# matvogel/P2P-Bridge

Hardware: AMD Instinct MI355X
Metric: denoised points/sec (8192-pt patches, T=30) (higher is better)
Workload: dtype f32; 1 GPU; PVDS_PUNet xyz-only, 8192-pt patches, T=30 bridge steps, batch 32 per GPU (BASELINE configs[1]); patches_per_gpu=32, points_per_patch=8192, bridge_steps=30, parallelism=patch-shard x1, process_group_world_size=1, hipgraph=True, weights=seeded random init (26.44 M params)

## Files before the change

### p2p_bridge_amd/csrc/common.h

```cpp
#pragma once
#include <hip/hip_runtime.h>
#include <stdint.h>
#include <type_traits>

#include "../../include/p2pb_hip.h"

#define P2PB_WAVE 64

static inline int p2pb_launch_status() { return (int)hipGetLastError(); }
int p2pb_split_terms_now();
#define p2pb_g_split_terms (p2pb_split_terms_now())

static inline unsigned cdiv(long a, long b) { return (unsigned)((a + b - 1) / b); }

template <int... Vs, class F>
static inline int for_value(int v, F &&f) {
  int rc = P2PB_EINVAL;
  (void)((v == Vs && (rc = f(std::integral_constant<int, Vs>{}), true)) || ...);
  return rc;
}
template <class F>
static inline int for_flag(bool v, F &&f) {
  return v ? f(std::true_type{}) : f(std::false_type{});
}

__device__ __forceinline__ float sqdist3(float dx, float dy, float dz) {
  return __fmaf_rn(dz, dz, __fmaf_rn(dy, dy, dx * dx));
}

__device__ __forceinline__ int lane_id() { return (int)(threadIdx.x & 63); }

__device__ __forceinline__ int mbcnt(unsigned long long mask) {
  return (int)__builtin_amdgcn_mbcnt_hi((unsigned)(mask >> 32), __builtin_amdgcn_mbcnt_lo((unsigned)mask, 0u));
}

template <int CTRL, int ROW_MASK>
__device__ __forceinline__ float dpp_add_step(float v) {
  const int o = __builtin_amdgcn_update_dpp(0, __builtin_bit_cast(int, v), CTRL, ROW_MASK, 0xf, false);
  return v + __builtin_bit_cast(float, o);
}
__device__ __forceinline__ float halfwave_sum_to_last(float v) {
  v = dpp_add_step<0x111, 0xf>(v);
  v = dpp_add_step<0x112, 0xf>(v);
  v = dpp_add_step<0x114, 0xf>(v);
  v = dpp_add_step<0x118, 0xf>(v);
  v = dpp_add_step<0x142, 0xa>(v);
  return v;
}

typedef __bf16 bf16x8 __attribute__((ext_vector_type(8)));
typedef __bf16 bf16x2 __attribute__((ext_vector_type(2)));
typedef float f32x2 __attribute__((ext_vector_type(2)));
typedef unsigned u32x4 __attribute__((ext_vector_type(4)));
typedef float f32x16 __attribute__((ext_vector_type(16)));

__device__ __forceinline__ void split3(float a, float b, unsigned &p0, unsigned &p1, unsigned &p2) {
  f32x2 v = {a, b};
  const bf16x2 q0 = __builtin_convertvector(v, bf16x2);
  v = v - __builtin_convertvector(q0, f32x2);
  const bf16x2 q1 = __builtin_convertvector(v, bf16x2);
  v = v - __builtin_convertvector(q1, f32x2);
  const bf16x2 q2 = __builtin_convertvector(v, bf16x2);
  p0 = __builtin_bit_cast(unsigned, q0);
  p1 = __builtin_bit_cast(unsigned, q1);
  p2 = __builtin_bit_cast(unsigned, q2);
}

#define SPLIT_BF16X6 6
#define SPLIT_BF16X3 3
#define SPLIT_F16X3 16
#define SPLIT_F16_SX 4.0f
typedef _Float16 f16x8 __attribute__((ext_vector_type(8)));
typedef _Float16 f16x2 __attribute__((ext_vector_type(2)));
__device__ __forceinline__ void split2h(float a, float b, unsigned &p0, unsigned &p1) {
  f32x2 v = {a, b};
  const f16x2 q0 = __builtin_convertvector(v, f16x2);
  v = v - __builtin_convertvector(q0, f32x2);
  const f16x2 q1 = __builtin_convertvector(v, f16x2);
  p0 = __builtin_bit_cast(unsigned, q0);
  p1 = __builtin_bit_cast(unsigned, q1);
}
template <int MODE>
__device__ __forceinline__ void split_pair(float a, float b, unsigned &p0, unsigned &p1, unsigned &p2) {
  if constexpr (MODE == SPLIT_F16X3) {
    split2h(a * SPLIT_F16_SX, b * SPLIT_F16_SX, p0, p1);
    p2 = 0u;
  } else {
    split3(a, b, p0, p1, p2);
  }
}
#define SPLIT_X2W_FLAG 0x100
#ifdef P2PB_X2W_TIMING
#define X2W_KEEP_LOW_WEIGHT_PRODUCT 0
#else
#define X2W_KEEP_LOW_WEIGHT_PRODUCT 1
#endif
constexpr __host__ __device__ int split_planes(int mode) { return mode == SPLIT_BF16X6 ? 3 : 2; }
template <int MODE>
__device__ __forceinline__ f32x16 split_mfma(const u32x4 &a, const u32x4 &b, const f32x16 &c) {
  if constexpr (MODE == SPLIT_F16X3)
    return __builtin_amdgcn_mfma_f32_32x32x16_f16(__builtin_bit_cast(f16x8, a), __builtin_bit_cast(f16x8, b), c, 0, 0, 0);
  else
    return __builtin_amdgcn_mfma_f32_32x32x16_bf16(__builtin_bit_cast(bf16x8, a), __builtin_bit_cast(bf16x8, b), c, 0, 0, 0);
}
__device__ __forceinline__ float f16_weight_scale(float wmax) {
  if (!(wmax > 0.0f) || wmax > 3.0e38f) return 1.0f;
  int e;
  (void)frexpf(wmax, &e);
  return ldexpf(1.0f, 14 - e);
}
struct GnFinish {
  const float *gamma, *beta, *style;
  float *scale, *shift, *chmean;
  double count_per_channel;
  int style_stride, groups;
  float eps;
};
static inline bool gn_shape_ok(int c, int groups, const float *style, int style_stride) {
  return groups > 0 && c % groups == 0 && c / groups <= 256 && !(style && style_stride < 2 * c);
}
typedef float gnf_f32x2 __attribute__((ext_vector_type(2)));
__device__ __forceinline__ void gn_finish_group_v(int c, int nslots, const float *__restrict__ part, const GnFinish &f, int b, int g,
                                                  double *lds, int vt, bool live, float *mean_rstd = nullptr,
                                                  float *tab_scale = nullptr, float *tab_shift = nullptr, float *tab_mean = nullptr) {
  double *rs = lds, *rq = lds + 256, *chs = lds + 512, *chq = lds + 768;
  const int t = vt;
  const int cg = c / f.groups, g0 = g * cg;
  const int nt = 256 / cg;
  const int k = t % cg, j = t / cg;
  float p_ga = 1.0f, p_be = 0.0f, p_fa = 1.0f, p_bi = 0.0f;
  if (live && t < cg) {
    const int ch = g0 + t;
    if (f.gamma) p_ga = f.gamma[ch];
    if (f.beta) p_be = f.beta[ch];
    if (f.style) {
      p_fa = f.style[(size_t)b * f.style_stride + ch];
      p_bi = f.style[(size_t)b * f.style_stride + c + ch];
    }
  }
  double s = 0.0, q = 0.0;
  if (live && j < nt) {
    const float *p0 = part + ((size_t)b * nslots * c + g0 + k) * 2;
    const size_t pitch = (size_t)c * 2;
    int sl = j;
    for (; sl + 7 * nt < nslots; sl += 8 * nt) {
      gnf_f32x2 v[8];
#pragma unroll
      for (int u = 0; u < 8; ++u) {
        const float *pp = p0 + (size_t)(sl + u * nt) * pitch;
        v[u] = *(const gnf_f32x2 *)pp;
      }
#pragma unroll
      for (int u = 0; u < 8; ++u) {
        s += (double)v[u][0];
        q += (double)v[u][1];
      }
    }
    for (; sl + 3 * nt < nslots; sl += 4 * nt) {
      gnf_f32x2 v[4];
#pragma unroll
      for (int u = 0; u < 4; ++u) {
        const float *pp = p0 + (size_t)(sl + u * nt) * pitch;
        v[u] = *(const gnf_f32x2 *)pp;
      }
#pragma unroll
      for (int u = 0; u < 4; ++u) {
        s += (double)v[u][0];
        q += (double)v[u][1];
      }
    }
    for (; sl < nslots; sl += nt) {
      const float *p = p0 + (size_t)sl * pitch;
      s += (double)p[0];
      q += (double)p[1];
    }
  }
  if (live) {
    rs[t] = s;
    rq[t] = q;
  }
  __syncthreads();
  if (live && t < cg) {
    double ts = 0.0, tq = 0.0;
    for (int jj = 0; jj < nt; ++jj) {
      ts += rs[jj * cg + t];
      tq += rq[jj * cg + t];
    }
    chs[t] = ts;
    chq[t] = tq;
  }
  __syncthreads();
  if (live && t < cg) {
    double gs = 0.0, gq = 0.0;
    for (int kk = 0; kk < cg; ++kk) {
      gs += chs[kk];
      gq += chq[kk];
    }
    const int ch = g0 + t;
    const double n = f.count_per_channel * cg;
    const double mean = gs / n;
    double var = gq / n - mean * mean;
    if (var < 0.0) var = 0.0;
    const double rstd = 1.0 / sqrt(var + (double)f.eps);
    const double ga = (double)p_ga, be = (double)p_be, fa = (double)p_fa, bi = (double)p_bi;
    const double sc = rstd * ga * fa;
    const double sh = (be - mean * rstd * ga) * fa + bi;
    const float cm = (float)(sc * (chs[t] / f.count_per_channel) + sh);
    if (f.scale) f.scale[(size_t)b * c + ch] = (float)sc;
    if (f.shift) f.shift[(size_t)b * c + ch] = (float)sh;
    if (f.chmean) f.chmean[(size_t)b * c + ch] = cm;
    if (tab_scale) tab_scale[ch] = (float)sc;
    if (tab_shift) tab_shift[ch] = (float)sh;
    if (tab_mean) tab_mean[ch] = cm;
    if (mean_rstd && t == 0) {
      mean_rstd[((size_t)b * f.groups + g) * 2] = (float)mean;
      mean_rstd[((size_t)b * f.groups + g) * 2 + 1] = (float)rstd;
    }
  }
  __syncthreads();
}
__device__ __forceinline__ void gn_finish_group(int c, int nslots, const float *__restrict__ part, const GnFinish &f, int b, int g,
                                                double *lds, float *mean_rstd = nullptr) {
  gn_finish_group_v(c, nslots, part, f, b, g, lds, (int)threadIdx.x, threadIdx.x < 256, mean_rstd);
}
template <int NS>
__device__ __forceinline__ void gn_finish_sample(int c, int nslots, const float *__restrict__ part, const GnFinish &f, int b, double *lds,
                                                 float *tab_scale = nullptr, float *tab_shift = nullptr, float *tab_mean = nullptr) {
  const int slice = (int)threadIdx.x >> 8, vt = (int)threadIdx.x & 255;
  for (int g0 = 0; g0 < f.groups; g0 += NS) {
    const int g = g0 + slice;
    gn_finish_group_v(c, nslots, part, f, b, g < f.groups ? g : 0, lds + slice * 1024, vt, slice < NS && g < f.groups, nullptr,
                      tab_scale, tab_shift, tab_mean);
  }
}
template <int CTRL>
__device__ __forceinline__ float dpp_full(float v) {
  const int i = __builtin_bit_cast(int, v);
  return __builtin_bit_cast(float, __builtin_amdgcn_update_dpp(i, i, CTRL, 0xf, 0xf, false));
}
__device__ __forceinline__ void permlane16_swap(float &a, float &b) {
  asm volatile("s_nop 1\n\tv_permlane16_swap_b32 %0, %1\n\ts_nop 1" : "+v"(a), "+v"(b));
}
struct RowAdd {
  __device__ static float f(float a, float b) { return a + b; }
};
__device__ __forceinline__ float vmin_raw(float a, float b) {
  float r;
  asm("v_min_f32 %0, %1, %2" : "=v"(r) : "v"(a), "v"(b));
  return r;
}
__device__ __forceinline__ float vmax_raw(float a, float b) {
  float r;
  asm("v_max_f32 %0, %1, %2" : "=v"(r) : "v"(a), "v"(b));
  return r;
}
struct RowMin {
  __device__ static float f(float a, float b) {
    float r;
    asm("v_min_f32 %0, %1, %2" : "=v"(r) : "v"(a), "v"(b));
    return r;
  }
};
struct RowMax {
  __device__ static float f(float a, float b) {
    float r;
    asm("v_max_f32 %0, %1, %2" : "=v"(r) : "v"(a), "v"(b));
    return r;
  }
};
template <class Op>
__device__ __forceinline__ float rowreduce32(float (&v)[32]) {
  const int lane = (int)(threadIdx.x & 63);
#pragma unroll
  for (int i = 0; i < 16; ++i) {
    float a = v[i], b = v[i + 16];
    permlane16_swap(a, b);
    v[i] = Op::f(a, b);
  }
#pragma unroll
  for (int i = 0; i < 8; ++i) {
    const float x = Op::f(v[i], dpp_full<0x128>(v[i])), y = Op::f(v[i + 8], dpp_full<0x128>(v[i + 8]));
    v[i] = (lane & 8) ? y : x;
  }
#pragma unroll
  for (int i = 0; i < 4; ++i) {
    const float x = Op::f(v[i], dpp_full<0x141>(v[i])), y = Op::f(v[i + 4], dpp_full<0x141>(v[i + 4]));
    v[i] = (lane & 4) ? y : x;
  }
#pragma unroll
  for (int i = 0; i < 2; ++i) {
    const float x = Op::f(v[i], dpp_full<0x4E>(v[i])), y = Op::f(v[i + 2], dpp_full<0x4E>(v[i + 2]));
    v[i] = (lane & 2) ? y : x;
  }
  const float x = Op::f(v[0], dpp_full<0xB1>(v[0])), y = Op::f(v[1], dpp_full<0xB1>(v[1]));
  return (lane & 1) ? y : x;
}

template <class Op>
__device__ __forceinline__ void groupreduce8(float (&v)[32]) {
  const int lane = (int)(threadIdx.x & 63);
#pragma unroll
  for (int i = 0; i < 16; ++i) {
    const float x = Op::f(v[i], dpp_full<0x141>(v[i])), y = Op::f(v[i + 16], dpp_full<0x141>(v[i + 16]));
    v[i] = (lane & 4) ? y : x;
  }
#pragma unroll
  for (int i = 0; i < 8; ++i) {
    const float x = Op::f(v[i], dpp_full<0x4E>(v[i])), y = Op::f(v[i + 8], dpp_full<0x4E>(v[i + 8]));
    v[i] = (lane & 2) ? y : x;
  }
#pragma unroll
  for (int i = 0; i < 4; ++i) {
    const float x = Op::f(v[i], dpp_full<0xB1>(v[i])), y = Op::f(v[i + 4], dpp_full<0xB1>(v[i + 4]));
    v[i] = (lane & 1) ? y : x;
  }
}

template <class Op>
__device__ __forceinline__ void groupreduce16(float (&v)[32]) {
  const int lane = (int)(threadIdx.x & 63);
#pragma unroll
  for (int i = 0; i < 16; ++i) {
    const float x = Op::f(v[i], dpp_full<0x140>(v[i])), y = Op::f(v[i + 16], dpp_full<0x140>(v[i + 16]));
    v[i] = (lane & 8) ? y : x;
  }
#pragma unroll
  for (int i = 0; i < 8; ++i) {
    const float x = Op::f(v[i], dpp_full<0x141>(v[i])), y = Op::f(v[i + 8], dpp_full<0x141>(v[i + 8]));
    v[i] = (lane & 4) ? y : x;
  }
#pragma unroll
  for (int i = 0; i < 4; ++i) {
    const float x = Op::f(v[i], dpp_full<0x4E>(v[i])), y = Op::f(v[i + 4], dpp_full<0x4E>(v[i + 4]));
    v[i] = (lane & 2) ? y : x;
  }
#pragma unroll
  for (int i = 0; i < 2; ++i) {
    const float x = Op::f(v[i], dpp_full<0xB1>(v[i])), y = Op::f(v[i + 2], dpp_full<0xB1>(v[i + 2]));
    v[i] = (lane & 1) ? y : x;
  }
}

enum {
  P2PB_FORM_PW_FP32 = 0,
  P2PB_FORM_PW_WIDE_FP32 = 1,
  P2PB_FORM_PW_WIDE_F16 = 2,
  P2PB_FORM_PW_SPLIT128 = 3,
  P2PB_FORM_PW_SPLIT256 = 4,
  P2PB_FORM_PW_PINGPONG = 5,
  P2PB_FORM_PW_GATHER = 6,
};
void p2pb_note_pointwise_form(int cin, int cout, int npos, int form);
int p2pb_gn_affine_launch(int b, int c, int nslots, const float *part, const GnFinish &f, hipStream_t s);

long p2pb_experiment_long(const char *key, long dflt);

int p2pb_zero_async(void *p, size_t nbytes, hipStream_t s);

bool p2pb_deterministic();
```

### p2p_bridge_amd/csrc/pointwise.hip

```cpp
#include "pw_common.h"
#include "absmax.h"

__global__ void pw_pack_kernel(int cout, int cin, int cin_pad, int cout_pad, const float *__restrict__ w,
                               float *__restrict__ wp, long s_co, long s_ci) {
  const size_t total = (size_t)cin_pad * cout_pad;
  for (size_t e = (size_t)blockIdx.x * 256 + threadIdx.x; e < total; e += (size_t)gridDim.x * 256) {
    const int kk = (int)(e & 3);
    const int co = (int)((e >> 2) % cout_pad);
    const int kh = (int)((e / ((size_t)4 * cout_pad)) & 1);
    const int chunk = (int)(e / ((size_t)8 * cout_pad));
    const int ci = chunk * 8 + 2 * kk + kh;
    wp[e] = (co < cout && ci < cin) ? w[(size_t)co * s_co + (size_t)ci * s_ci] : 0.0f;
  }
}

extern "C" size_t p2pb_pointwise_packed_floats(int cout, int cin) {
  return (size_t)pw_cin_pad(cin) * pw_cout_pad(cout);
}

static int pw_pack(int cout, int cin, const float *w, float *wp, bool adjoint, void *stream) {
  if (cout <= 0 || cin <= 0) return P2PB_EINVAL;
  const size_t total = p2pb_pointwise_packed_floats(cout, cin);
  hipLaunchKernelGGL(pw_pack_kernel, dim3((unsigned)((total + 255) / 256 > 2048 ? 2048 : (total + 255) / 256)), dim3(256),
                     0, (hipStream_t)stream, cout, cin, pw_cin_pad(cin), pw_cout_pad(cout), w, wp, adjoint ? 1L : (long)cin,
                     adjoint ? (long)cout : 1L);
  return p2pb_launch_status();
}
extern "C" int p2pb_pointwise_pack_weights(int cout, int cin, const float *w, float *wp, void *stream) {
  return pw_pack(cout, cin, w, wp, false, stream);
}
extern "C" int p2pb_pointwise_pack_weights_adjoint(int cout, int cin, const float *w_forward, float *wp, void *stream) {
  return pw_pack(cout, cin, w_forward, wp, true, stream);
}

__global__ void pw_pack_split_kernel(int cout, int cin, int nchunk, int ncoblk, const float *__restrict__ w,
                                     unsigned short *__restrict__ wp, int mode, float *__restrict__ trailer, long s_co, long s_ci,
                                     const unsigned *__restrict__ amax) {
  const size_t total = (size_t)nchunk * ncoblk * 2 * 2 * 128 * 8;
  const bool x2w = (mode & SPLIT_X2W_FLAG) != 0;
  mode &= 0xff;
  const float wmax = amax ? __builtin_bit_cast(float, *amax) : trailer[0];
  const float sw = mode == SPLIT_F16X3 ? f16_weight_scale(wmax) : 1.0f;
  if (blockIdx.x == 0 && threadIdx.x == 0) {
    trailer[1] = mode == SPLIT_F16X3 ? 1.0f / (SPLIT_F16_SX * sw) : 1.0f;
    if (amax) trailer[0] = wmax, trailer[2] = trailer[3] = 0.0f;
  }
  for (size_t e = (size_t)blockIdx.x * 256 + threadIdx.x; e < total; e += (size_t)gridDim.x * 256) {
    const int idx = (int)(e & 7);
    size_t q = e >> 3;
    const int col = (int)(q & 127);
    q >>= 7;
    const int kh = (int)(q & 1);
    q >>= 1;
    const int ks = (int)(q & 1);
    q >>= 1;
    const int cb = (int)(q % ncoblk), chunk = (int)(q / ncoblk);
    const int co = cb * 128 + col, ci = chunk * PWS_CK + ks * 16 + kh * 8 + idx;
    const float x = (co < cout && ci < cin) ? w[(size_t)co * s_co + (size_t)ci * s_ci] : 0.0f;
    unsigned p0, p1, p2;
    if (mode == SPLIT_F16X3) {
      split2h(x * sw, 0.0f, p0, p1);
      if (x2w) p1 = 0u;
      p2 = 0u;
    } else {
      split3(x, 0.0f, p0, p1, p2);
    }
    const unsigned pp[3] = {p0, p1, p2};
    for (int s = 0; s < 3; ++s)
      wp[((((((size_t)chunk * ncoblk + cb) * 2 + ks) * 3 + s) * 2 + kh) * 128 + col) * 8 + idx] = (unsigned short)(pp[s] & 0xffff);
  }
}

extern "C" size_t p2pb_pointwise_split_packed_bytes(int cout, int cin) {
  const size_t nchunk = (cin + PWS_CK - 1) / PWS_CK, ncoblk = (cout + 127) / 128;
  return nchunk * ncoblk * (2 * 3 * 2 * 128) * 16 + 16;
}

static int pw_pack_split(int cout, int cin, const float *w, void *wp, bool adjoint, void *stream, const unsigned *amax = nullptr) {
  if (cout <= 0 || cin <= 0) return P2PB_EINVAL;
  const int nchunk = (cin + PWS_CK - 1) / PWS_CK, ncoblk = (cout + 127) / 128;
  const size_t total = (size_t)nchunk * ncoblk * 2 * 2 * 128 * 8;
  float *trailer = (float *)((char *)wp + (size_t)nchunk * ncoblk * PWS_TILE * 16);
  static const long x2w = p2pb_experiment_long("x2w", 0);
  const int mode = p2pb_g_split_terms;
  if (mode == SPLIT_F16X3 && !amax) {
    const int rc = p2pb_zero_async(trailer, 16, (hipStream_t)stream);
    if (rc) return rc;
    hipLaunchKernelGGL(absmax_bits_kernel, dim3(absmax_blocks((size_t)cout * cin)), dim3(256), 0, (hipStream_t)stream, w, (size_t)cout * cin,
                       (unsigned *)trailer);
  }
  hipLaunchKernelGGL(pw_pack_split_kernel, dim3((unsigned)((total + 255) / 256 > 2048 ? 2048 : (total + 255) / 256)),
                     dim3(256), 0, (hipStream_t)stream, cout, cin, nchunk, ncoblk, w, (unsigned short *)wp,
                     mode | ((x2w && mode == SPLIT_F16X3 && !adjoint) ? SPLIT_X2W_FLAG : 0), trailer,
                     adjoint ? 1L : (long)cin, adjoint ? (long)cout : 1L, mode == SPLIT_F16X3 ? amax : nullptr);
  return p2pb_launch_status();
}
extern "C" int p2pb_pointwise_pack_weights_split(int cout, int cin, const float *w, void *wp, void *stream) {
  return pw_pack_split(cout, cin, w, wp, false, stream);
}
extern "C" int p2pb_pointwise_pack_weights_split_adjoint(int cout, int cin, const float *w_forward, void *wp, void *stream) {
  return pw_pack_split(cout, cin, w_forward, wp, true, stream);
}
extern "C" int p2pb_pointwise_pack_weights_split_amax(int cout, int cin, const float *w, void *wp, const unsigned *amax_bits,
                                                      void *stream) {
  return amax_bits ? pw_pack_split(cout, cin, w, wp, false, stream, amax_bits) : P2PB_EINVAL;
}

static GnFinish pw_fin(double count_per_channel, int groups, const float *gamma, const float *beta, const float *style,
                       int style_stride, float eps, float *scale, float *shift, float *chmean) {
  GnFinish f = {};
  f.gamma = gamma, f.beta = beta, f.style = style, f.scale = scale, f.shift = shift, f.chmean = chmean;
  f.count_per_channel = count_per_channel, f.style_stride = style_stride, f.groups = groups, f.eps = eps;
  return f;
}
static bool pw_fin_ok(const GnFinish &f, int cout, const float *stats_part) {
  return !f.scale || (stats_part && f.shift && f.count_per_channel > 0.0 && gn_shape_ok(cout, f.groups, f.style, f.style_stride));
}
static int pw_finish_behind(int rc, int b, int cout, int P, const float *stats_part, const GnFinish &f, hipStream_t s) {
  if (rc != 0 || !f.scale) return rc;
  return p2pb_gn_affine_launch(b, cout, (P + 255) / 256 * 4, stats_part, f, s);
}

static int pw_run_split(const PwArgs &a) {
  const int mode = p2pb_g_split_terms;
  static const int wm_env = (int)p2pb_experiment_long("pw_wm", 0);
  const bool wm4 = !a.out_pm && (wm_env ? wm_env == 4
                                         : (a.cout >= 512 && (long)((a.P + 127) / 128) * ((a.cout + 255) / 256) * a.b >= 1024));
  if (mode == SPLIT_BF16X3 && (a.in_scale || a.minmax || a.out_pm)) return P2PB_EINVAL;
  static const int pp_env = (int)p2pb_experiment_long("pw_pp", 1);
  if (pp_env && wm4 && mode == SPLIT_F16X3 && a.cin % 64 == 0 && a.cout % 512 == 0 && (!a.minmax || a.pool_u == 0) &&
      (size_t)a.cin * a.P * 4 < (1ull << 31)) {
    p2pb_note_pointwise_form(a.cin, a.cout, a.P, P2PB_FORM_PW_PINGPONG);
    return pw_pp512_launch(a);
  }
  p2pb_note_pointwise_form(a.cin, a.cout, a.P, wm4 ? P2PB_FORM_PW_SPLIT256 : P2PB_FORM_PW_SPLIT128);
  return pw_split_launch(a, mode, wm4);
}

static int pw_run(const PwArgs &a, int flags) {
  const bool rows16 = pw_wide_ok(a.P, a.in, a.out);
  if ((flags & PW_SPLIT_PACK) && (flags & PW_WIDE_TILING)) {
    if (!rows16 || p2pb_g_split_terms != SPLIT_F16X3) return P2PB_EINVAL;
    p2pb_note_pointwise_form(a.cin, a.cout, a.P, P2PB_FORM_PW_WIDE_F16);
    return pw_wide_f16_launch(a);
  }
  if (flags & PW_SPLIT_PACK) return rows16 ? pw_run_split(a) : P2PB_EINVAL;
  if (rows16) {
    p2pb_note_pointwise_form(a.cin, a.cout, a.P, P2PB_FORM_PW_WIDE_FP32);
    return pw_wide_fp32_launch(a);
  }
  if (a.minmax || a.out_pm) return P2PB_EINVAL;
  p2pb_note_pointwise_form(a.cin, a.cout, a.P, P2PB_FORM_PW_FP32);
  return pw_conv_launch(a);
}

extern "C" size_t p2pb_pointwise_stats_floats(int b, int cout, int npos) {
  return (size_t)b * ((npos + 255) / 256) * 4 * cout * 2;
}

extern "C" int p2pb_pointwise_conv_forward(int b, int cin, int cout, int npos, const float *in, const void *wp_any,
                                           const float *bias, const float *bias_b, const float *in_scale,
                                           const float *in_shift, int in_swish, int flags, float *out,
                                           float *stats_part, double fin_count_per_channel, int fin_groups,
                                           const float *fin_gamma, const float *fin_beta, const float *fin_style,
                                           int fin_style_stride, float fin_eps, float *fin_scale, float *fin_shift,
                                           float *fin_chmean, void *stream) {
  const GnFinish f = pw_fin(fin_count_per_channel, fin_groups, fin_gamma, fin_beta, fin_style, fin_style_stride, fin_eps, fin_scale,
                            fin_shift, fin_chmean);
  if (!pw_fin_ok(f, cout, stats_part)) return P2PB_EINVAL;
  if (b <= 0 || cin <= 0 || cout <= 0 || npos <= 0 || !out) return P2PB_EINVAL;
  const int out_pm = (flags & PW_OUT_POINT_MAJOR) != 0;
  if (out_pm && stats_part) return P2PB_EINVAL;
  const PwArgs a = {b,   cin,        cout,    npos, in,     wp_any, bias, bias_b, in_scale, in_shift, in_swish,
                    out, stats_part, nullptr, 0,    out_pm, (hipStream_t)stream};
  return pw_finish_behind(pw_run(a, flags), b, cout, npos, stats_part, f, a.s);
}

extern "C" int p2pb_pointwise_pool_supported(int npos, int pool_u) {
  const bool uok = pool_u == 0 || pool_u == 4 || pool_u == 8 || pool_u == 16 || pool_u == 32 || pool_u == 64;
  return npos > 0 && npos % 4 == 0 && uok && (pool_u == 0 || npos % pool_u == 0);
}

extern "C" size_t p2pb_pointwise_minmax_floats(int b, int cout, int npos, int pool_u, int flags) {
  const bool split_tiling = (flags & PW_SPLIT_PACK) && !(flags & PW_WIDE_TILING);
  if (pool_u == 0) return (size_t)b * (split_tiling ? (npos + 127) / 128 * 2 : (npos + 511) / 512 * 4) * cout * 2;
  return (size_t)b * cout * (npos / pool_u) * 2;
}

extern "C" int p2pb_pointwise_conv_pool_forward(int b, int cin, int cout, int npos, const float *in,
                                                const void *wp_any, const float *bias, const float *bias_b,
                                                const float *in_scale, const float *in_shift, int in_swish, int flags,
                                                float *out, float *stats_part, int pool_u, float *minmax,
                                                double fin_count_per_channel, int fin_groups, const float *fin_gamma,
                                                const float *fin_beta, const float *fin_style, int fin_style_stride,
                                                float fin_eps, float *fin_scale, float *fin_shift, float *fin_chmean,
                                                void *stream) {
  const GnFinish f = pw_fin(fin_count_per_channel, fin_groups, fin_gamma, fin_beta, fin_style, fin_style_stride, fin_eps, fin_scale,
                            fin_shift, fin_chmean);
  if (!pw_fin_ok(f, cout, stats_part)) return P2PB_EINVAL;
  if (b <= 0 || cin <= 0 || cout <= 0 || npos <= 0 || !minmax || !stats_part) return P2PB_EINVAL;
  if (!p2pb_pointwise_pool_supported(npos, pool_u) || !pw_wide_ok(npos, in, out)) return P2PB_EINVAL;
  const PwArgs a = {b,   cin,        cout,   npos,   in, wp_any, bias, bias_b, in_scale, in_shift, in_swish,
                    out, stats_part, minmax, pool_u, 0,  (hipStream_t)stream};
  return pw_finish_behind(pw_run(a, flags), b, cout, npos, stats_part, f, a.s);
}

extern "C" int p2pb_pointwise_conv_pool_gather(int b, int cin, int cout, int n, int m, int u, const float *zt,
                                               const float *cxt, const int *idx, const void *wp_split, const float *bias,
                                               const float *in_scale, const float *in_shift, int in_swish,
                                               float *stats_part, float *minmax, double fin_count_per_channel,
                                               int fin_groups, const float *fin_gamma, const float *fin_beta,
                                               const float *fin_style, int fin_style_stride, float fin_eps, float *fin_scale,
                                               float *fin_shift, float *fin_chmean, void *stream) {
  const GnFinish f = pw_fin(fin_count_per_channel, fin_groups, fin_gamma, fin_beta, fin_style, fin_style_stride, fin_eps, fin_scale,
                            fin_shift, fin_chmean);
  const long npos = (long)m * u;
  if (b <= 0 || cin <= 0 || cout <= 0 || n <= 0 || m <= 0 || !zt || !idx || !wp_split || !in_scale || !in_shift ||
      !stats_part || !minmax || (cin & 7) || npos > 0x7fffffffL || !p2pb_pointwise_pool_supported((int)npos, u) || u == 0 ||
      p2pb_g_split_terms != SPLIT_F16X3 || (((uintptr_t)zt | (uintptr_t)cxt) & 15) || !pw_fin_ok(f, cout, stats_part))
    return P2PB_EINVAL;
  const PwArgs a = {b,       cin,        cout,   (int)npos, zt, wp_split, bias, nullptr, in_scale, in_shift, in_swish,
                    nullptr, stats_part, minmax, u,         0,  (hipStream_t)stream};
  p2pb_note_pointwise_form(cin, cout, a.P, P2PB_FORM_PW_GATHER);
  return pw_finish_behind(pw_gather_launch(a, PwGather{cxt, idx, n, u}), b, cout, a.P, stats_part, f, a.s);
}
```

### p2p_bridge_amd/csrc/pw_common.h

```cpp
#pragma once
#include "common.h"

typedef float f32x4 __attribute__((ext_vector_type(4)));

__device__ __forceinline__ float swishf(float v) {
  return v * __builtin_amdgcn_rcpf(1.0f + __builtin_amdgcn_exp2f(v * -1.44269504088896340736f));
}

template <int CTRL, int ROW_MASK>
__device__ __forceinline__ float dpp_perm(float v) {
  const int i = __builtin_bit_cast(int, v);
  return __builtin_bit_cast(float, __builtin_amdgcn_update_dpp(i, i, CTRL, ROW_MASK, 0xf, false));
}
__device__ __forceinline__ void group_minmax(float &mn, float &mx, int g) {
  if (g > 1) { mn = vmin_raw(mn, dpp_perm<0xB1, 0xf>(mn)); mx = vmax_raw(mx, dpp_perm<0xB1, 0xf>(mx)); }
  if (g > 2) { mn = vmin_raw(mn, dpp_perm<0x4E, 0xf>(mn)); mx = vmax_raw(mx, dpp_perm<0x4E, 0xf>(mx)); }
  if (g > 4) { mn = vmin_raw(mn, dpp_perm<0x141, 0xf>(mn)); mx = vmax_raw(mx, dpp_perm<0x141, 0xf>(mx)); }
  if (g > 8) { mn = vmin_raw(mn, dpp_perm<0x140, 0xf>(mn)); mx = vmax_raw(mx, dpp_perm<0x140, 0xf>(mx)); }
  if (g > 16) { mn = vmin_raw(mn, dpp_perm<0x142, 0xa>(mn)); mx = vmax_raw(mx, dpp_perm<0x142, 0xa>(mx)); }
}

static inline int pw_cin_pad(int cin) { return (cin + 7) / 8 * 8; }
static inline int pw_cout_pad(int cout) { return (cout + 127) / 128 * 128; }
#define PWS_CK 32
#define PWS_TILE (2 * 3 * 2 * 128)
static inline int pw_nslots(int P) { return (P + 255) / 256 * 4; }

static bool pw_wide_ok(int P, const float *in, const float *out) {
  return P % 4 == 0 && (((uintptr_t)in | (uintptr_t)out) & 15) == 0;
}

static int pool_lanes(int pool_u) { return pool_u == 0 ? 32 : pool_u / 4; }

enum {
  PW_SPLIT_PACK = 4,
  PW_OUT_POINT_MAJOR = 32,
  PW_WIDE_TILING = 128,
};

struct PwGather {
  const float *cxt;
  const int *idx;
  int gn, gu;
};

struct PwArgs {
  int b, cin, cout, P;
  const float *in;
  const void *wp;
  const float *bias, *bias_b, *in_scale, *in_shift;
  int in_swish;
  float *out, *stats_part;
  float *minmax;
  int pool_u;
  int out_pm;
  hipStream_t s;
};

template <class F>
static inline int pw_for_mt(int cout, F &&f) {
  return cout > 32 ? f(std::integral_constant<int, 2>{}) : f(std::integral_constant<int, 1>{});
}

int pw_conv_launch(const PwArgs &a);
int pw_wide_fp32_launch(const PwArgs &a);
int pw_wide_f16_launch(const PwArgs &a);
int pw_gather_launch(const PwArgs &a, const PwGather &gat);
int pw_split_launch(const PwArgs &a, int terms, bool wm4);
int pw_pp512_launch(const PwArgs &a);
```

Baseline: 1.184 million points/s.

## Add K-split pointwise conv kernel for small-grid deep-channel layers

Adds a split-K pointwise convolution kernel in which the four waves of a block each process interleaved input-channel stages and then reduce their accumulators through LDS before a shared epilogue. It is selected for the F16x3 split path when cin is at least 192 and the normal 128x128 tile grid would have fewer than 256 blocks, using smaller 64x64 output tiles. The aim is to raise occupancy and parallelism for low-resolution, high-channel layers that otherwise underfill the GPU. The cost is an extra LDS reduction, a barrier, and an epilogue run by a single wave per block.

```diff
diff --git a/p2p_bridge_amd/csrc/common.h b/p2p_bridge_amd/csrc/common.h
--- a/p2p_bridge_amd/csrc/common.h
+++ b/p2p_bridge_amd/csrc/common.h
@@ -349,6 +349,7 @@
   P2PB_FORM_PW_SPLIT256 = 4,
   P2PB_FORM_PW_PINGPONG = 5,
   P2PB_FORM_PW_GATHER = 6,
+  P2PB_FORM_PW_KSPLIT = 7,
 };
 void p2pb_note_pointwise_form(int cin, int cout, int npos, int form);
 int p2pb_gn_affine_launch(int b, int c, int nslots, const float *part, const GnFinish &f, hipStream_t s);
diff --git a/p2p_bridge_amd/csrc/pointwise.hip b/p2p_bridge_amd/csrc/pointwise.hip
--- a/p2p_bridge_amd/csrc/pointwise.hip
+++ b/p2p_bridge_amd/csrc/pointwise.hip
@@ -133,6 +133,12 @@
     p2pb_note_pointwise_form(a.cin, a.cout, a.P, P2PB_FORM_PW_PINGPONG);
     return pw_pp512_launch(a);
   }
+  static const int ks_env = (int)p2pb_experiment_long("pw_ksplit", 1);
+  if (ks_env && !wm_env && mode == SPLIT_F16X3 && !a.out_pm && a.cin >= 192 &&
+      (long)((a.P + 127) / 128) * ((a.cout + 127) / 128) * a.b < 256) {
+    p2pb_note_pointwise_form(a.cin, a.cout, a.P, P2PB_FORM_PW_KSPLIT);
+    return pw_ksplit_launch(a);
+  }
   p2pb_note_pointwise_form(a.cin, a.cout, a.P, wm4 ? P2PB_FORM_PW_SPLIT256 : P2PB_FORM_PW_SPLIT128);
   return pw_split_launch(a, mode, wm4);
 }
diff --git a/p2p_bridge_amd/csrc/pointwise_ksplit.hip b/p2p_bridge_amd/csrc/pointwise_ksplit.hip
--- /dev/null
+++ b/p2p_bridge_amd/csrc/pointwise_ksplit.hip
@@ -0,0 +1,16 @@
+#include "pw_ksplit.h"
+
+template <bool XF, int PL>
+static int pw_ksplit_go(const PwArgs &a) {
+  const dim3 grid((a.P + 127) / 128 * 2, (a.cout + 63) / 64, a.b);
+  hipLaunchKernelGGL((pw_ksplit_kernel<XF, PL>), grid, dim3(256), PWK_LDS_BYTES, a.s, a.cin, a.cout, a.P, pw_nslots(a.P), a.in,
+                     (const u32x4 *)a.wp, a.bias, a.bias_b, a.in_scale, a.in_shift, a.in_swish, a.out, a.stats_part, a.minmax,
+                     a.pool_u);
+  return p2pb_launch_status();
+}
+int pw_ksplit_launch(const PwArgs &a) {
+  const int pl = !a.minmax ? 0 : a.pool_u == 0 ? 1 : a.pool_u == 32 ? 32 : 2;
+  return for_flag(a.in_scale != nullptr, [&](auto XF) {
+    return for_value<0, 1, 32, 2>(pl, [&](auto PL) { return pw_ksplit_go<XF(), PL()>(a); });
+  });
+}
diff --git a/p2p_bridge_amd/csrc/pw_common.h b/p2p_bridge_amd/csrc/pw_common.h
--- a/p2p_bridge_amd/csrc/pw_common.h
+++ b/p2p_bridge_amd/csrc/pw_common.h
@@ -68,3 +68,4 @@
 int pw_gather_launch(const PwArgs &a, const PwGather &gat);
 int pw_split_launch(const PwArgs &a, int terms, bool wm4);
 int pw_pp512_launch(const PwArgs &a);
+int pw_ksplit_launch(const PwArgs &a);
diff --git a/p2p_bridge_amd/csrc/pw_ksplit.h b/p2p_bridge_amd/csrc/pw_ksplit.h
--- /dev/null
+++ b/p2p_bridge_amd/csrc/pw_ksplit.h
@@ -0,0 +1,172 @@
+#pragma once
+#include "pw_split.h"
+
+#define PWK_A_STAGE (2 * 2 * 2 * 64)
+#define PWK_WAVE_LDS (2 * PWK_A_STAGE)
+#define PWK_LDS_BYTES (4 * PWK_WAVE_LDS * 16)
+
+template <bool XF, int PL>
+__global__ __launch_bounds__(256, 2) void pw_ksplit_kernel(int cin, int cout, int P, int nslots, const float *__restrict__ in,
+                                                            const u32x4 *__restrict__ wp, const float *__restrict__ bias,
+                                                            const float *__restrict__ bias_b,
+                                                            const float *__restrict__ in_scale,
+                                                            const float *__restrict__ in_shift, int in_swish,
+                                                            float *__restrict__ out, float *__restrict__ stats_part,
+                                                            float *__restrict__ mm_out, int pool_u) {
+  extern __shared__ u32x4 pwk_lds[];
+  constexpr int TERMS = SPLIT_F16X3;
+  const int tid = threadIdx.x, lane = tid & 63;
+  const int wave = __builtin_amdgcn_readfirstlane(tid >> 6);
+  const int l31 = lane & 31, khalf = lane >> 5;
+  const int ncoblk = gridDim.y;
+  const unsigned lin = blockIdx.x + gridDim.x * (blockIdx.y + gridDim.y * blockIdx.z);
+  const unsigned nblk = gridDim.x * gridDim.y * gridDim.z;
+  const unsigned vid = nblk % 8 == 0 ? (lin % 8) * (nblk / 8) + lin / 8 : lin;
+  const int bx = (vid / ncoblk) % gridDim.x, by = vid % ncoblk;
+  const int b = vid / (ncoblk * gridDim.x);
+  const int p0 = bx * 64, co0 = by * 64;
+  const int nblk128 = (cout + 127) / 128, nstage = (cin + PWS_CK - 1) / PWS_CK;
+  const float *inb = in + (size_t)b * cin * P;
+  const bool work = p0 < P;
+  u32x4 *lds_w = pwk_lds + wave * PWK_WAVE_LDS;
+
+  f32x16 acc[2][2];
+#pragma unroll
+  for (int m = 0; m < 2; ++m)
+#pragma unroll
+    for (int n = 0; n < 2; ++n)
+#pragma unroll
+      for (int r = 0; r < 16; ++r) acc[m][n][r] = 0.0f;
+
+  const int pl = p0 + 2 * l31;
+  const float *inl = inb + (pl < P ? pl : P - 2);
+  float braw[2][8][2], xsc[2][8], xsh[2][8];
+  auto load_b = [&](int st) {
+#pragma unroll
+    for (int ks = 0; ks < 2; ++ks)
+#pragma unroll
+      for (int i = 0; i < 8; ++i) {
+        const int row = min(st * PWS_CK + ks * 16 + khalf * 8 + i, cin - 1);
+        const f32x2 v = *(const f32x2 *)(inl + (size_t)row * P);
+        braw[ks][i][0] = v[0];
+        braw[ks][i][1] = v[1];
+        if (XF) {
+          xsc[ks][i] = in_scale[b * cin + row];
+          xsh[ks][i] = in_shift[b * cin + row];
+        }
+      }
+  };
+  auto dma_a = [&](int st, int buf) {
+    const u32x4 *src = wp + ((size_t)st * nblk128 + (by >> 1)) * PWS_TILE + (by & 1) * 64 + lane;
+    u32x4 *dst = lds_w + buf * PWK_A_STAGE;
+#pragma unroll
+    for (int ks = 0; ks < 2; ++ks)
+#pragma unroll
+      for (int s = 0; s < 2; ++s)
+#pragma unroll
+        for (int kh = 0; kh < 2; ++kh)
+          __builtin_amdgcn_global_load_lds((const __attribute__((address_space(1))) void *)(src + ((ks * 3 + s) * 2 + kh) * 128),
+                                           (__attribute__((address_space(3))) void *)(dst + ((ks * 2 + s) * 2 + kh) * 64), 16, 0, 0);
+  };
+
+  if (work && wave < nstage) {
+    dma_a(wave, 0);
+    load_b(wave);
+  }
+  int buf = 0;
+  for (int st = wave; work && st < nstage; st += 4, buf ^= 1) {
+    asm volatile("s_waitcnt vmcnt(0)" ::: "memory");
+    u32x4 bf[2][2][2];
+#pragma unroll
+    for (int ks = 0; ks < 2; ++ks) {
+      if (XF) {
+#pragma unroll
+        for (int i = 0; i < 8; ++i)
+#pragma unroll
+          for (int e = 0; e < 2; ++e) {
+            float v = braw[ks][i][e] * xsc[ks][i] + xsh[ks][i];
+            if (in_swish) v = swishf(v);
+            braw[ks][i][e] = v;
+          }
+      }
+#pragma unroll
+      for (int e = 0; e < 2; ++e)
+#pragma unroll
+        for (int i = 0; i < 4; ++i) {
+          unsigned q0, q1, q2;
+          split_pair<TERMS>(braw[ks][2 * i][e], braw[ks][2 * i + 1][e], q0, q1, q2);
+          bf[ks][0][e][i] = q0;
+          bf[ks][1][e][i] = q1;
+        }
+    }
+    if (st + 4 < nstage) {
+      dma_a(st + 4, buf ^ 1);
+      load_b(st + 4);
+    }
+    const u32x4 *la = lds_w + buf * PWK_A_STAGE;
+#pragma unroll
+    for (int ks = 0; ks < 2; ++ks) {
+      u32x4 af[2][2];
+#pragma unroll
+      for (int s = 0; s < 2; ++s)
+#pragma unroll
+        for (int m = 0; m < 2; ++m) af[s][m] = la[((ks * 2 + s) * 2 + khalf) * 64 + m * 32 + l31];
+      constexpr int PA[3] = {1, 0, 0}, PB[3] = {0, 1, 0};
+#pragma unroll
+      for (int t = 0; t < 3; ++t)
+#pragma unroll
+        for (int m = 0; m < 2; ++m)
+#pragma unroll
+          for (int n = 0; n < 2; ++n)
+            if (X2W_KEEP_LOW_WEIGHT_PRODUCT || PA[t] != 1) acc[m][n] = split_mfma<TERMS>(af[PA[t]][m], bf[ks][PB[t]][n], acc[m][n]);
+    }
+  }
+
+  float *sb = (float *)pwk_lds;
+  if (wave == 0) {
+    const int co = co0 + lane;
+    float v = 0.0f;
+    if (co < cout) {
+      v = bias ? bias[co] : 0.0f;
+      if (bias_b) v += bias_b[(size_t)b * cout + co];
+    }
+    sb[lane] = v;
+  } else {
+#pragma unroll
+    for (int m = 0; m < 2; ++m)
+#pragma unroll
+      for (int n = 0; n < 2; ++n)
+#pragma unroll
+        for (int j = 0; j < 4; ++j)
+          lds_w[((m * 2 + n) * 4 + j) * 64 + lane] = __builtin_bit_cast(
+              u32x4, f32x4{acc[m][n][4 * j], acc[m][n][4 * j + 1], acc[m][n][4 * j + 2], acc[m][n][4 * j + 3]});
+  }
+  __syncthreads();
+  if (wave != 0) return;
+  const float oscale = ((const float *)(wp + (size_t)nstage * nblk128 * PWS_TILE))[1];
+#pragma unroll
+  for (int w = 1; w < 4; ++w) {
+#pragma unroll
+    for (int m = 0; m < 2; ++m)
+#pragma unroll
+      for (int n = 0; n < 2; ++n)
+#pragma unroll
+        for (int j = 0; j < 4; ++j) {
+          const f32x4 v = __builtin_bit_cast(f32x4, pwk_lds[w * PWK_WAVE_LDS + ((m * 2 + n) * 4 + j) * 64 + lane]);
+#pragma unroll
+          for (int i = 0; i < 4; ++i) acc[m][n][4 * j + i] += v[i];
+        }
+#pragma unroll
+    for (int m = 0; m < 2; ++m)
+#pragma unroll
+      for (int n = 0; n < 2; ++n) asm volatile("" : "+v"(acc[m][n]));
+  }
+#pragma unroll
+  for (int m = 0; m < 2; ++m)
+#pragma unroll
+    for (int n = 0; n < 2; ++n)
+#pragma unroll
+      for (int r = 0; r < 16; ++r) acc[m][n][r] *= oscale;
+  pws_epilogue<PL, 2, 1>(acc, b, bx >> 1, (int)gridDim.x >> 1, (bx >> 1) * 128, co0, 0, bx & 1, l31, khalf, cout, P, nslots, bias,
+                         bias_b, out, stats_part, mm_out, pool_u, 0, sb);
+}
```

Result: no change. 1.193 million points/s (median of 6 runs) (+0.7%).
